# livesense-inc/fanlin-rs

Hardware: AMD Instinct MI355X
Metric: images/sec whole-node (1080p→300×200 resize+encode); p50 per-image ms (higher is better)
Workload: dtype u8 (exact, as f16 subnormals) x the reference's f32 weights as three f16 terms -> f32 sums (vertical, v_mfma_f32_16x16x32_f16); 24-bit fixed-point intermediate (2^-14 steps, three i8 planes) x 24-bit fixed-point weights (2^-24 steps, three i8 digits), eight of the nine digit products -> exact i32 (h

## Files before the change

### fanlin-rs_amd/csrc/fl_jpeg.hip

```cpp
#include <hip/hip_runtime.h>
#include <stdint.h>

#include "fl_jpeg.h"
#include "fl_jpeg_tables.h"
#include "fl_pixel.h"
#include "fl_types.h"

namespace fl {

namespace {


constexpr int32_t F_0_298 = 2446, F_0_390 = 3196, F_0_541 = 4433, F_0_765 = 6270, F_0_899 = 7373, F_1_175 = 9633, F_1_501 = 12299,
                  F_1_847 = 15137, F_1_961 = 16069, F_2_053 = 16819, F_2_562 = 20995, F_3_072 = 25172;

struct Mat8 { int32_t a[8][8]; };

constexpr void fdct_linear(const int32_t in[8], int32_t out[8])
{
    int32_t t0 = in[0] + in[7], t1 = in[1] + in[6], t2 = in[2] + in[5], t3 = in[3] + in[4];
    const int32_t t10 = t0 + t3, t11 = t1 + t2;
    int32_t t12 = t0 - t3, t13 = t1 - t2;
    t0 = in[0] - in[7]; t1 = in[1] - in[6]; t2 = in[2] - in[5]; t3 = in[3] - in[4];
    out[0] = t10 + t11;
    out[4] = t10 - t11;
    int32_t z1 = (t12 + t13) * F_0_541;
    out[2] = z1 + t12 * F_0_765;
    out[6] = z1 - t13 * F_1_847;
    t12 = t0 + t2;
    t13 = t1 + t3;
    z1 = (t12 + t13) * F_1_175;
    t12 = t12 * (-F_0_390) + z1;
    t13 = t13 * (-F_1_961) + z1;
    z1 = (t0 + t3) * (-F_0_899);
    out[1] = t0 * F_1_501 + z1 + t12;
    out[7] = t3 * F_0_298 + z1 + t13;
    z1 = (t1 + t2) * (-F_2_562);
    out[3] = t1 * F_3_072 + z1 + t13;
    out[5] = t2 * F_2_053 + z1 + t12;
}

constexpr Mat8 make_fdct_matrix()
{
    Mat8 m{};
    for (int j = 0; j < 8; ++j) {
        int32_t e[8] = {0, 0, 0, 0, 0, 0, 0, 0}, o[8] = {0, 0, 0, 0, 0, 0, 0, 0};
        e[j] = 1;
        fdct_linear(e, o);
        for (int k = 0; k < 8; ++k) m.a[k][j] = o[k];
    }
    return m;
}

__constant__ Mat8 kFdct = make_fdct_matrix();

constexpr bool fdct_matrix_fits_i16()
{
    const Mat8 m = make_fdct_matrix();
    for (int k = 0; k < 8; ++k)
        for (int j = 0; j < 8; ++j)
            if (m.a[k][j] > 32767 || m.a[k][j] < -32768) return false;
    return true;
}
static_assert(fdct_matrix_fits_i16(), "the passes use v_dot2_i32_i16: matrix entries must be 16-bit");

typedef short i16x2 __attribute__((ext_vector_type(2)));
__device__ __forceinline__ i16x2 as_i16x2(uint32_t v) { return __builtin_bit_cast(i16x2, v); }
__device__ __forceinline__ uint32_t pack_i16(int32_t lo, int32_t hi) { return ((uint32_t)lo & 0xffffu) | ((uint32_t)hi << 16); }
__device__ __forceinline__ int32_t dot8_i16(const uint32_t m[4], const uint4 v)
{
    int32_t p = __builtin_amdgcn_sdot2(as_i16x2(m[0]), as_i16x2(v.x), 0, false);
    p = __builtin_amdgcn_sdot2(as_i16x2(m[1]), as_i16x2(v.y), p, false);
    p = __builtin_amdgcn_sdot2(as_i16x2(m[2]), as_i16x2(v.z), p, false);
    return __builtin_amdgcn_sdot2(as_i16x2(m[3]), as_i16x2(v.w), p, false);
}

struct NaturalOrder { uint8_t n[64]; };
constexpr NaturalOrder make_natural()
{
    NaturalOrder t{};
    for (int k = 0; k < 64; ++k) t.n[k] = kUnzigzag[k];
    return t;
}
__constant__ NaturalOrder kNatural = make_natural();

struct HuffLut { uint32_t e[256]; };

constexpr HuffLut make_lut(const HuffSpec &s)
{
    HuffLut t{};
    uint32_t code = 0;
    int k = 0;
    for (int l = 1; l <= 16; ++l) {
        for (int i = 0; i < s.len[l - 1]; ++i, ++k) t.e[s.val[k]] = ((uint32_t)l << 16) | code++;
        code <<= 1;
    }
    return t;
}

struct HuffAll { HuffLut ac[2], dc[2]; };
constexpr HuffAll make_all() { return HuffAll{{make_lut(kAcLuma), make_lut(kAcChroma)}, {make_lut(kDcLuma), make_lut(kDcChroma)}}; }
__constant__ HuffAll kHuff = make_all();


template <int N>
__device__ __forceinline__ uint32_t dpp_row_shr(uint32_t v)
{
    return (uint32_t)__builtin_amdgcn_update_dpp(0, (int)v, 0x110 + N, 0xf, 0xf, false);
}

__device__ __forceinline__ uint32_t wave_inclusive_scan(uint32_t v, uint32_t lane)
{
    (void)lane;
    v += dpp_row_shr<1>(v);
    v += dpp_row_shr<2>(v);
    v += dpp_row_shr<4>(v);
    v += dpp_row_shr<8>(v);
    v += (uint32_t)__builtin_amdgcn_update_dpp(0, (int)v, 0x142, 0xa, 0xf, false);
    v += (uint32_t)__builtin_amdgcn_update_dpp(0, (int)v, 0x143, 0xc, 0xf, false);
    return v;
}

__device__ __forceinline__ void wave_lds_sync()
{
    __builtin_amdgcn_fence(__ATOMIC_SEQ_CST, "wavefront");
    __builtin_amdgcn_wave_barrier();
}

constexpr uint32_t kPackThreads = 512;
constexpr uint32_t kPackWaves = kPackThreads / 64;

__device__ __forceinline__ uint32_t wg_exclusive_scan(uint32_t v, uint32_t *s_w, uint32_t *total)
{
    const uint32_t lane = threadIdx.x & 63u, wave = threadIdx.x >> 6;
    const uint32_t inc = wave_inclusive_scan(v, lane);
    __syncthreads();
    if (lane == 63u) s_w[wave] = inc;
    __syncthreads();
    uint32_t base = 0, sum = 0;
#pragma unroll
    for (uint32_t i = 0; i < kPackWaves; ++i) { const uint32_t t = s_w[i]; if (i < wave) base += t; sum += t; }
    *total = sum;
    return base + inc - v;
}

__device__ __forceinline__ uint32_t coef_size(int32_t v)
{
    const uint32_t mag = (uint32_t)(v < 0 ? -v : v);
    return mag ? 32u - (uint32_t)__clz(mag) : 0u;
}


#ifndef FL_JPEG_BPW
#define FL_JPEG_BPW 16
#define FL_JPEG_WPG 2
#define FL_JPEG_PREFETCH 3
#endif
constexpr uint32_t kBlocksPerWave = FL_JPEG_BPW;
constexpr uint32_t kWavesPerWg = FL_JPEG_WPG;
constexpr uint32_t kPrefetch = FL_JPEG_PREFETCH;
static_assert(kBlocksPerWave == 32u || kBlocksPerWave == 16u, "the coding phase's lane mapping");
constexpr uint32_t kJpegThreads = 64u * kWavesPerWg;
constexpr uint32_t kBlocksPerWg = kWavesPerWg * kBlocksPerWave;
constexpr uint32_t kUnitsPerWave = 3u * kBlocksPerWave;

static_assert(63u * (16u + 10u) <= kAcWordsPerUnit * 32u, "a unit's AC code must fit its acbits slot");

struct WaveLds {
    int16_t coef[kUnitsPerWave][64];
    uint64_t nz[kUnitsPerWave];
    __attribute__((aligned(16))) int16_t smp[3][64];
    __attribute__((aligned(16))) int16_t p1[3][64];
};

__device__ __forceinline__ void stage_ac_luts(uint32_t *s_ac)
{
    for (uint32_t i = threadIdx.x; i < 512u; i += kJpegThreads) s_ac[i] = kHuff.ac[i >> 8].e[i & 255u];
    __syncthreads();
}

template <bool kRgba>
__device__ __forceinline__ uint32_t block_pixel(const JpegJob &jb, uint32_t brow, uint32_t bcol, uint32_t r, uint32_t c)
{
    uint32_t px = bcol * 8u + c, py = brow * 8u + r;
    px = px < jb.w ? px : jb.w - 1u;
    py = py < jb.h ? py : jb.h - 1u;
    if constexpr (kRgba) return ((const __attribute__((address_space(1))) uint32_t *)jb.src)[(size_t)py * jb.w + px];
    uint32_t pr, pg, pb, pa;
    load_rgba(jb.src + ((size_t)py * jb.w + px) * jb.c, jb.c, pr, pg, pb, pa);
    return pr | (pg << 8) | (pb << 16);
}

__device__ __forceinline__ void dct_quant_block(const uint32_t (&smp)[3], uint32_t nat, uint32_t r, uint32_t c, const uint32_t (&m1)[4],
                                                const uint32_t (&m2)[4], uint4 k1, const uint32_t (&q)[3], const uint32_t (&magic)[3],
                                                WaveLds &w, int32_t (&qv)[3])
{
#pragma unroll
    for (int k = 0; k < 3; ++k) w.smp[k][nat] = (int16_t)smp[k];
    wave_lds_sync();
#pragma unroll
    for (int k = 0; k < 3; ++k) {
        const int32_t p = dot8_i16(m1, *reinterpret_cast<const uint4 *>(w.smp[k] + r * 8));
        const int32_t v1 = ((p << k1.x) + (int32_t)k1.y) >> 11;
        w.p1[k][c * 8 + r] = (int16_t)v1;
    }
    wave_lds_sync();
#pragma unroll
    for (int k = 0; k < 3; ++k) {
        const int32_t p2 = dot8_i16(m2, *reinterpret_cast<const uint4 *>(w.p1[k] + c * 8));
        const int32_t d = (p2 + (int32_t)k1.z) >> k1.w;
        const int32_t sg = d >> 31;
        const uint32_t an = (uint32_t)((d ^ sg) - sg) >> 3;
        const uint32_t rq = __umulhi(2u * an + q[k], magic[k]);
        qv[k] = ((int32_t)rq ^ sg) - sg;
    }
}

typedef __attribute__((address_space(1))) uint32_t global_u32;

struct UnitBits {
    uint64_t acc;
    uint32_t pend, total, wi;
    global_u32 *out;
    __device__ __forceinline__ void put(uint32_t code, uint32_t len)
    {
        acc = (acc << len) | code;
        pend += len;
        total += len;
        if (pend >= 32u) { pend -= 32u; out[wi++] = (uint32_t)(acc >> pend); }
    }
};

template <bool kRgba>
__device__ __forceinline__ void transform_blocks(const JpegJob &jb, const uint32_t *__restrict__ arena, uint32_t first, uint32_t count,
                                                 uint32_t lane, WaveLds &w)
{
    const uint32_t nat = kNatural.n[lane], r = nat >> 3, c = nat & 7u;
    uint32_t m1[4], m2[4];
#pragma unroll
    for (int j = 0; j < 4; ++j) {
        m1[j] = pack_i16(kFdct.a[c][2 * j], kFdct.a[c][2 * j + 1]);
        m2[j] = pack_i16(kFdct.a[r][2 * j], kFdct.a[r][2 * j + 1]);
    }
    const uint8_t *qt = reinterpret_cast<const uint8_t *>(arena + jb.tab_off) + 624;
    const uint32_t *mg = reinterpret_cast<const uint32_t *>(qt + 128);
    const uint32_t q[3] = {qt[nat], qt[64 + nat], qt[64 + nat]};
    const uint32_t magic[3] = {mg[nat], mg[64 + nat], mg[64 + nat]};
    const uint4 k1 = {(c == 0u || c == 4u) ? 13u : 0u, c == 0u ? (uint32_t)(-(8 * 128) * 8192) : (c == 4u ? 0u : 1u << 10),
                      (r == 0u || r == 4u) ? 2u : 1u << 14, (r == 0u || r == 4u) ? 2u : 15u};
    uint32_t brow = first / jb.bx, bcol = first - brow * jb.bx;
    uint32_t ahead[kPrefetch];
#pragma unroll
    for (uint32_t j = 0; j < kPrefetch; ++j) {
        ahead[j] = block_pixel<kRgba>(jb, brow, bcol, r, c);
        if (++bcol == jb.bx) { bcol = 0; ++brow; }
    }
    for (uint32_t i = 0; i < count; ++i) {
        const uint32_t rgb = kRgba ? ahead[0] & 0xffffffu : ahead[0];
#pragma unroll
        for (uint32_t j = 0; j + 1u < kPrefetch; ++j) ahead[j] = ahead[j + 1u];
        ahead[kPrefetch - 1u] = block_pixel<kRgba>(jb, brow, bcol, r, c);
        if (++bcol == jb.bx) { bcol = 0; ++brow; }
        uint32_t smp[3];
        jfif_px(rgb, smp[0], smp[1], smp[2]);
        const bool flat = __ballot(rgb != (uint32_t)__builtin_amdgcn_readfirstlane((int)rgb)) == 0ull;
        if (flat) {
            if (lane == 0u) {
#pragma unroll
                for (int k = 0; k < 3; ++k) {
                    const int32_t d = 64 * ((int32_t)smp[k] - 128);
                    const int32_t sg = d >> 31;
                    const uint32_t an = (uint32_t)((d ^ sg) - sg) >> 3;
                    const uint32_t rq = __umulhi(2u * an + q[k], magic[k]);
                    w.coef[i * 3u + k][0] = (int16_t)(((int32_t)rq ^ sg) - sg);
                    w.nz[i * 3u + k] = 0ull;
                }
            }
            continue;
        }
        int32_t qv[3];
        dct_quant_block(smp, nat, r, c, m1, m2, k1, q, magic, w, qv);
#pragma unroll
        for (int k = 0; k < 3; ++k) {
            w.coef[i * 3u + k][lane] = (int16_t)qv[k];
            const uint64_t nz = __ballot(qv[k] != 0) & ~1ull;
            if (lane == 0u) w.nz[i * 3u + k] = nz;
        }
    }
}

__global__ __launch_bounds__(kJpegThreads) void jpeg_dct_quant_kernel(const JpegJob *__restrict__ jobs, const uint32_t *__restrict__ arena,
                                                                      uint32_t job_base)
{
    __shared__ WaveLds s_w[kWavesPerWg];
    __shared__ uint32_t s_ac[512];
    const JpegJob jb = jobs[job_base + blockIdx.y];
    const uint32_t wave = threadIdx.x >> 6, lane = threadIdx.x & 63u;
    const uint32_t nblocks = jb.bx * jb.by;
    if (blockIdx.x * kBlocksPerWg >= nblocks) return;
    stage_ac_luts(s_ac);
    const uint32_t first = blockIdx.x * kBlocksPerWg + wave * kBlocksPerWave;
    if (first >= nblocks) return;
    const uint32_t count = min(kBlocksPerWave, nblocks - first);
    WaveLds &w = s_w[wave];

    if (jb.c == 4u && (reinterpret_cast<uintptr_t>(jb.src) & 3u) == 0u) transform_blocks<true>(jb, arena, first, count, lane, w);
    else transform_blocks<false>(jb, arena, first, count, lane, w);
    wave_lds_sync();

    uint32_t b, u, u_end;
    bool chroma;
    if constexpr (kBlocksPerWave == 32u) {
        b = lane & 31u;
        chroma = lane >= 32u;
        u = b * 3u + (chroma ? 1u : 0u);
        u_end = b * 3u + (chroma ? 3u : 1u);
    } else {
        b = lane & 15u;
        chroma = lane >= 16u;
        u = b * 3u + (lane >> 4);
        u_end = lane >= 48u ? u : u + 1u;
    }
    if (b >= count) return;
    const uint32_t *tab = s_ac + (chroma ? 256u : 0u);
    const uint32_t eob = tab[0], zrl = tab[0xF0];
    for (; u < u_end; ++u) {
        const uint32_t unit = first * 3u + u;
        const int16_t *cf = w.coef[u];
        uint64_t m = w.nz[u];
        UnitBits ub{0ull, 0u, 0u, unit * kAcWordsPerUnit, (global_u32 *)jb.acbits};
        uint32_t prev = 0;
        uint32_t pos = (uint32_t)__builtin_ctzll(m | (1ull << 63));
        int32_t v = cf[pos];
        while (m) {
            const uint32_t cpos = pos;
            const int32_t cv = v;
            m &= m - 1ull;
            pos = (uint32_t)__builtin_ctzll(m | (1ull << 63));
            v = cf[pos];
            uint32_t run = cpos - prev - 1u;
            prev = cpos;
            while (run > 15u) { ub.put(zrl & 0xffffu, zrl >> 16); run -= 16u; }
            const uint32_t mag = (uint32_t)(cv < 0 ? -cv : cv);
            const uint32_t size = 32u - (uint32_t)__clz(mag);
            const uint32_t value = (uint32_t)(cv + (cv >> 31)) & ((1u << size) - 1u);
            const uint32_t e = tab[(run << 4) | size];
            ub.put(((e & 0xffffu) << size) | value, (e >> 16) + size);
        }
        if (prev != 63u) ub.put(eob & 0xffffu, eob >> 16);
        if (ub.pend) ub.out[ub.wi] = (uint32_t)(ub.acc << (32u - ub.pend));
        jb.meta[unit] = ((uint32_t)(uint16_t)cf[0]) | (ub.total << 16);
    }
}


constexpr uint32_t kWinWords = 8192;

__device__ __forceinline__ void win_or(uint32_t *win, uint32_t wbase, uint64_t g, uint32_t val)
{
    const uint64_t W = g >> 5;
    const uint32_t sh = (uint32_t)g & 31u;
    const uint32_t hi = val >> sh, lo = sh ? val << (32u - sh) : 0u;
    if (hi && W >= wbase && W < (uint64_t)wbase + kWinWords) atomicOr(&win[W - wbase], hi);
    if (lo && W + 1 >= wbase && W + 1 < (uint64_t)wbase + kWinWords) atomicOr(&win[W + 1 - wbase], lo);
}

__device__ __forceinline__ uint32_t dc_code(const JpegJob &jb, uint32_t u, uint32_t meta, uint32_t *len)
{
    const int32_t dc = (int16_t)(meta & 0xffffu), prev = u >= 3u ? (int32_t)(int16_t)(jb.meta[u - 3u] & 0xffffu) : 0;
    const int32_t diff = dc - prev;
    const uint32_t size = coef_size(diff);
    const uint32_t value = (uint32_t)(diff < 0 ? diff - 1 : diff) & ((1u << size) - 1u);
    const uint32_t e = kHuff.dc[(u % 3u) ? 1 : 0].e[size];
    *len = (e >> 16) + size;
    return (((e & 0xffffu) << size) | value) << (32u - *len);
}

__global__ __launch_bounds__(kPackThreads) void jpeg_pack_kernel(const JpegJob *__restrict__ jobs, const uint32_t *__restrict__ arena,
                                                                 uint32_t job_base)
{
    __shared__ uint32_t s_win[kWinWords];
    __shared__ uint32_t s_w[kPackWaves], s_carry, s_lo, s_hi;
    const JpegJob jb = jobs[job_base + blockIdx.x];
    const uint32_t tid = threadIdx.x;
    const uint32_t nunits = jb.bx * jb.by * 3u;
    constexpr uint32_t T = kPackThreads;

    for (uint32_t i = tid; i < kWinWords; i += T) s_win[i] = 0u;
    if (tid == 0u) s_carry = 0u;
    __syncthreads();
    for (uint32_t base = 0; base < nunits; base += T) {
        const uint32_t u = base + tid;
        uint32_t len = 0, dl = 0, dcw = 0, nw = 0, a0 = 0, a1 = 0;
        if (u < nunits) {
            const uint32_t m = jb.meta[u];
            nw = ((m >> 16) + 31u) >> 5;
            if (nw > 0u) a0 = jb.acbits[(size_t)u * kAcWordsPerUnit];
            if (nw > 1u) a1 = jb.acbits[(size_t)u * kAcWordsPerUnit + 1u];
            dcw = dc_code(jb, u, m, &dl);
            len = dl + (m >> 16);
        }
        uint32_t chunk;
        const uint32_t ex = wg_exclusive_scan(len, s_w, &chunk);
        const uint32_t carry = s_carry;
        if (u < nunits) {
            const uint32_t off = carry + ex;
            jb.unit_off[u] = off;
            win_or(s_win, 0u, off, dcw);
            if (nw > 0u) win_or(s_win, 0u, (uint64_t)off + dl, a0);
            if (nw > 1u) win_or(s_win, 0u, (uint64_t)off + dl + 32u, a1);
            for (uint32_t w = 2; w < nw; ++w) win_or(s_win, 0u, (uint64_t)off + dl + 32u * w, jb.acbits[(size_t)u * kAcWordsPerUnit + w]);
        }
        __syncthreads();
        if (tid == 0u) s_carry = carry + chunk;
        __syncthreads();
    }
    const uint32_t total_bits = s_carry;
    if (tid == 0u) jb.unit_off[nunits] = total_bits;
    __threadfence_block();
    __syncthreads();
    const uint32_t nbytes = (total_bits + 7u) >> 3, limit = jb.dst_cap;
    const uint8_t *hdr = reinterpret_cast<const uint8_t *>(arena + jb.tab_off);
    for (uint32_t i = tid; i < kJpegHeaderBytes; i += T) if (i < limit) jb.dst[i] = hdr[i];

    uint32_t ff_before = 0;
    for (uint32_t wbase = 0; wbase * 32ull < total_bits; wbase += kWinWords) {
        const uint64_t wb = (uint64_t)wbase * 32u, we = wb + (uint64_t)kWinWords * 32u;
        if (wbase != 0u) {
            for (uint32_t i = tid; i < kWinWords; i += T) s_win[i] = 0u;
            if (tid == 0u) {
                uint32_t lo = 0, hi = nunits;
                while (lo < hi) { const uint32_t mid = (lo + hi) >> 1; if (jb.unit_off[mid + 1u] > wb) hi = mid; else lo = mid + 1u; }
                s_lo = lo;
                uint32_t lo2 = lo, hi2 = nunits;
                while (lo2 < hi2) { const uint32_t mid = (lo2 + hi2) >> 1; if (jb.unit_off[mid] >= we) hi2 = mid; else lo2 = mid + 1u; }
                s_hi = lo2;
            }
        } else if (tid == 0u) { s_lo = 0u; s_hi = 0u; }
        __syncthreads();
        const uint32_t u_lo = s_lo, u_hi = s_hi;
        for (uint32_t ub = u_lo; ub < u_hi; ub += T / 2u) {
            const uint32_t u = ub + (tid >> 1), j = tid & 1u;
            if (u < u_hi) {
                const uint32_t m = jb.meta[u], off = jb.unit_off[u];
                uint32_t dl;
                const uint32_t dcw = dc_code(jb, u, m, &dl);
                if (j == 0u) win_or(s_win, wbase, off, dcw);
                const uint32_t nw = ((m >> 16) + 31u) >> 5;
                for (uint32_t w = j; w < nw; w += 2u)
                    win_or(s_win, wbase, (uint64_t)off + dl + 32u * w, jb.acbits[(size_t)u * kAcWordsPerUnit + w]);
            }
        }
        __syncthreads();
        if (tid == 0u && (total_bits & 7u) && (total_bits >> 5) >= wbase && (total_bits >> 5) < wbase + kWinWords)
            s_win[(total_bits >> 5) - wbase] |= (0xFFu >> (total_bits & 7u)) << (24u - 8u * ((total_bits >> 3) & 3u));
        __syncthreads();
        const uint32_t win_bytes = (uint32_t)min((uint64_t)kWinWords * 4u, (uint64_t)nbytes - (uint64_t)wbase * 4u);
        if (tid == 0u) s_carry = 0u;
        __syncthreads();
        for (uint32_t base = 0; base < win_bytes; base += 4u * T) {
            const uint32_t i = base + tid * 4u;
            const uint32_t word = i < win_bytes ? s_win[i >> 2] : 0u;
            const uint32_t valid = i < win_bytes ? (win_bytes - i < 4u ? win_bytes - i : 4u) : 0u;
            uint32_t ff = 0;
#pragma unroll
            for (uint32_t k = 0; k < 4; ++k) ff += (k < valid && ((word >> (24u - 8u * k)) & 255u) == 255u) ? 1u : 0u;
            uint32_t chunk;
            const uint32_t ex = wg_exclusive_scan(ff, s_w, &chunk);
            const uint32_t carry = s_carry;
            uint64_t o = (uint64_t)kJpegHeaderBytes + (uint64_t)wbase * 4u + i + ff_before + carry + ex;
#pragma unroll
            for (uint32_t k = 0; k < 4; ++k) {
                if (k < valid) {
                    const uint32_t b = (word >> (24u - 8u * k)) & 255u;
                    if (o < limit) jb.dst[o] = (uint8_t)b;
                    ++o;
                    if (b == 255u) { if (o < limit) jb.dst[o] = 0u; ++o; }
                }
            }
            __syncthreads();
            if (tid == 0u) s_carry = carry + chunk;
            __syncthreads();
        }
        ff_before += s_carry;
        __syncthreads();
    }
    if (tid == 0u) {
        const uint64_t end = (uint64_t)kJpegHeaderBytes + nbytes + ff_before;
        if (end + 2u <= limit) {
            jb.dst[end] = 0xFF; jb.dst[end + 1u] = 0xD9;
            jb.result[1] = (uint32_t)(end + 2u);
        } else {
            jb.result[1] = 0u;
            atomicOr(&jb.result[0], FL_JPEG_RESULT_OVERFLOW);
        }
    }
}

}

hipError_t launch_jpeg_encode(const JpegJob *jobs, const uint32_t *arena, uint32_t job_base, uint32_t njobs, uint32_t max_blocks,
                              hipStream_t st)
{
    if (!njobs || !max_blocks) return hipSuccess;
    hipLaunchKernelGGL(jpeg_dct_quant_kernel, dim3((max_blocks + kBlocksPerWg - 1) / kBlocksPerWg, njobs), dim3(kJpegThreads), 0, st, jobs, arena, job_base);
    FL_LAUNCH_CHECK();
    hipLaunchKernelGGL(jpeg_pack_kernel, dim3(njobs), dim3(kPackThreads), 0, st, jobs, arena, job_base);
    FL_LAUNCH_CHECK();
    return hipSuccess;
}

}
```

Baseline: 555,300.

## Restructure JPEG pack kernel: multi-unit-per-thread scans, fewer barriers, wave-level stuffing

Reworks the pack kernel so each thread handles six units and eight window words per round. Offsets come from wave-level scans, with a single cross-wave LDS exchange per round that uses double-buffered scratch, which removes most workgroup barriers and the tid-0 carry round-trips. It also counts 0xFF bytes with a bit trick, narrows addressing to 32-bit, preloads the DC Huffman tables into LDS, and uses 8-byte AC loads. Units with more than two AC words take a separate slow path. The cost is higher register pressure and more complex lane-to-component mapping logic.

```diff
diff --git a/fanlin-rs_amd/csrc/fl_jpeg.hip b/fanlin-rs_amd/csrc/fl_jpeg.hip
--- a/fanlin-rs_amd/csrc/fl_jpeg.hip
+++ b/fanlin-rs_amd/csrc/fl_jpeg.hip
@@ -130,18 +130,23 @@
 constexpr uint32_t kPackThreads = 512;
 constexpr uint32_t kPackWaves = kPackThreads / 64;
 
-__device__ __forceinline__ uint32_t wg_exclusive_scan(uint32_t v, uint32_t *s_w, uint32_t *total)
+__device__ __forceinline__ void lds_barrier()
+{
+    __builtin_amdgcn_fence(__ATOMIC_RELEASE, "workgroup", "local");
+    __builtin_amdgcn_s_barrier();
+    __builtin_amdgcn_fence(__ATOMIC_ACQUIRE, "workgroup", "local");
+}
+
+__device__ __forceinline__ uint32_t waves_exclusive_scan(uint32_t wave_total, uint32_t *s_w, uint32_t *total)
 {
     const uint32_t lane = threadIdx.x & 63u, wave = threadIdx.x >> 6;
-    const uint32_t inc = wave_inclusive_scan(v, lane);
-    __syncthreads();
-    if (lane == 63u) s_w[wave] = inc;
-    __syncthreads();
+    if (lane == 0u) s_w[wave] = wave_total;
+    lds_barrier();
     uint32_t base = 0, sum = 0;
 #pragma unroll
     for (uint32_t i = 0; i < kPackWaves; ++i) { const uint32_t t = s_w[i]; if (i < wave) base += t; sum += t; }
     *total = sum;
-    return base + inc - v;
+    return base;
 }
 
 __device__ __forceinline__ uint32_t coef_size(int32_t v)
@@ -355,141 +360,232 @@
 
 
 constexpr uint32_t kWinWords = 8192;
-
-__device__ __forceinline__ void win_or(uint32_t *win, uint32_t wbase, uint64_t g, uint32_t val)
-{
-    const uint64_t W = g >> 5;
-    const uint32_t sh = (uint32_t)g & 31u;
+constexpr uint32_t kPackUnitsPerThread = 6;
+constexpr uint32_t kPackWordsPerThread = 8;
+constexpr uint32_t kPackRoundUnits = kPackThreads * kPackUnitsPerThread;
+constexpr uint32_t kPackRoundWords = kPackThreads * kPackWordsPerThread;
+static_assert((64u * kPackUnitsPerThread) % 3u == 0u, "a wave's run of units starts with a Y unit: the component is (step + lane) % 3");
+static_assert(kWinWords % kPackRoundWords == 0u, "the stuffing rounds tile the window");
+static_assert(kAcWordsPerUnit % 2u == 0u, "a unit's first two AC words are one 8-byte load");
+constexpr uint32_t kPackHeaderPerThread = (kJpegHeaderBytes + kPackThreads - 1u) / kPackThreads;
+
+typedef __attribute__((address_space(1))) uint8_t global_u8;
+typedef uint32_t u32x2 __attribute__((ext_vector_type(2)));
+typedef __attribute__((address_space(1))) u32x2 global_u32x2;
+
+__device__ __forceinline__ uint32_t load_u32(const global_u32 *base, uint32_t byte_off)
+{
+    return *(const global_u32 *)((const global_u8 *)base + byte_off);
+}
+__device__ __forceinline__ void store_u32(global_u32 *base, uint32_t byte_off, uint32_t v)
+{
+    *(global_u32 *)((global_u8 *)base + byte_off) = v;
+}
+
+__device__ __forceinline__ void win_or(uint32_t *win, uint32_t wbase, uint32_t g, uint32_t val)
+{
+    const uint32_t W = (g >> 5) - wbase;
+    const uint32_t sh = g & 31u;
     const uint32_t hi = val >> sh, lo = sh ? val << (32u - sh) : 0u;
-    if (hi && W >= wbase && W < (uint64_t)wbase + kWinWords) atomicOr(&win[W - wbase], hi);
-    if (lo && W + 1 >= wbase && W + 1 < (uint64_t)wbase + kWinWords) atomicOr(&win[W + 1 - wbase], lo);
-}
-
-__device__ __forceinline__ uint32_t dc_code(const JpegJob &jb, uint32_t u, uint32_t meta, uint32_t *len)
-{
-    const int32_t dc = (int16_t)(meta & 0xffffu), prev = u >= 3u ? (int32_t)(int16_t)(jb.meta[u - 3u] & 0xffffu) : 0;
+    if (hi && W < kWinWords) atomicOr(&win[W], hi);
+    if (lo && W + 1u < kWinWords) atomicOr(&win[W + 1u], lo);
+}
+
+__device__ __forceinline__ uint32_t dc_code(int32_t dc, int32_t prev, const uint32_t *e, uint32_t *len)
+{
     const int32_t diff = dc - prev;
     const uint32_t size = coef_size(diff);
     const uint32_t value = (uint32_t)(diff < 0 ? diff - 1 : diff) & ((1u << size) - 1u);
-    const uint32_t e = kHuff.dc[(u % 3u) ? 1 : 0].e[size];
-    *len = (e >> 16) + size;
-    return (((e & 0xffffu) << size) | value) << (32u - *len);
-}
-
-__global__ __launch_bounds__(kPackThreads) void jpeg_pack_kernel(const JpegJob *__restrict__ jobs, const uint32_t *__restrict__ arena,
-                                                                 uint32_t job_base)
+    const uint32_t c = e[size];
+    *len = (c >> 16) + size;
+    return (((c & 0xffffu) << size) | value) << (32u - *len);
+}
+
+__device__ __forceinline__ uint32_t count_ff(uint32_t w)
+{
+    const uint32_t x = ~w;
+    return (uint32_t)__popc(~(((x & 0x7f7f7f7fu) + 0x7f7f7f7fu) | x | 0x7f7f7f7fu));
+}
+
+__global__ __launch_bounds__(kPackThreads) __attribute__((amdgpu_waves_per_eu(8, 8)))
+void jpeg_pack_kernel(const JpegJob *__restrict__ jobs, const uint32_t *__restrict__ arena, uint32_t job_base)
 {
     __shared__ uint32_t s_win[kWinWords];
-    __shared__ uint32_t s_w[kPackWaves], s_carry, s_lo, s_hi;
+    __shared__ uint32_t s_scan[2][kPackWaves], s_dc[2][16], s_lo, s_hi;
     const JpegJob jb = jobs[job_base + blockIdx.x];
-    const uint32_t tid = threadIdx.x;
+    const uint32_t tid = threadIdx.x, lane = tid & 63u, wave = tid >> 6;
     const uint32_t nunits = jb.bx * jb.by * 3u;
-    constexpr uint32_t T = kPackThreads;
-
-    for (uint32_t i = tid; i < kWinWords; i += T) s_win[i] = 0u;
-    if (tid == 0u) s_carry = 0u;
-    __syncthreads();
-    for (uint32_t base = 0; base < nunits; base += T) {
-        const uint32_t u = base + tid;
-        uint32_t len = 0, dl = 0, dcw = 0, nw = 0, a0 = 0, a1 = 0;
-        if (u < nunits) {
-            const uint32_t m = jb.meta[u];
-            nw = ((m >> 16) + 31u) >> 5;
-            if (nw > 0u) a0 = jb.acbits[(size_t)u * kAcWordsPerUnit];
-            if (nw > 1u) a1 = jb.acbits[(size_t)u * kAcWordsPerUnit + 1u];
-            dcw = dc_code(jb, u, m, &dl);
-            len = dl + (m >> 16);
+    constexpr uint32_t T = kPackThreads, U = kPackUnitsPerThread, S = kPackWordsPerThread;
+    const global_u32 *meta = (const global_u32 *)jb.meta;
+    const global_u32 *acw = (const global_u32 *)jb.acbits;
+    const global_u32x2 *ac2 = (const global_u32x2 *)jb.acbits;
+    global_u32 *unit_off = (global_u32 *)jb.unit_off;
+    global_u8 *dst = (global_u8 *)jb.dst;
+    const global_u8 *hdr = (const global_u8 *)(arena + jb.tab_off);
+    const uint32_t limit = jb.dst_cap;
+    uint32_t par = 0;
+
+    const uint32_t l3 = lane % 3u;
+    uint32_t carry = 0;
+    for (uint32_t base = 0; base < nunits; base += kPackRoundUnits) {
+        const uint32_t u0 = base + wave * (64u * U) + lane;
+        uint32_t m[U], mp[U];
+        u32x2 a[U];
+#pragma unroll
+        for (uint32_t s = 0; s < U; ++s) {
+            const uint32_t uc = min(u0 + 64u * s, nunits - 1u);
+            m[s] = load_u32(meta, uc * 4u);
+            mp[s] = load_u32(meta, (uc >= 3u ? uc - 3u : 0u) * 4u);
+            a[s] = __builtin_nontemporal_load(&ac2[(size_t)uc * (kAcWordsPerUnit / 2u)]);
+        }
+        if (base == 0u) {
+            for (uint32_t i = tid; i < kWinWords; i += T) s_win[i] = 0u;
+            const uint32_t dc_entry = kHuff.dc[(tid >> 4) & 1u].e[tid & 15u];
+            if (tid < 32u) s_dc[tid >> 4][tid & 15u] = dc_entry;
+            lds_barrier();
+        }
+        uint32_t dcw[U], info[U], ex[U], run = 0;
+        bool longer = false;
+#pragma unroll
+        for (uint32_t s = 0; s < U; ++s) {
+            const uint32_t u = u0 + 64u * s;
+            const bool chroma = l3 != (3u - s % 3u) % 3u;
+            const int32_t prev = u >= 3u ? (int32_t)(int16_t)(mp[s] & 0xffffu) : 0;
+            uint32_t dl;
+            dcw[s] = dc_code((int16_t)(m[s] & 0xffffu), prev, s_dc[chroma ? 1 : 0], &dl);
+            const uint32_t acl = u < nunits ? m[s] >> 16 : 0u;
+            const uint32_t len = u < nunits ? dl + acl : 0u;
+            info[s] = dl | (acl << 8);
+            longer |= acl > 64u;
+            const uint32_t inc = wave_inclusive_scan(len, lane);
+            ex[s] = run + inc - len;
+            run += (uint32_t)__builtin_amdgcn_readlane((int)inc, 63);
+            asm volatile("" : "+v"(dcw[s]), "+v"(info[s]), "+v"(ex[s]));
+            __builtin_amdgcn_sched_barrier(0);
         }
         uint32_t chunk;
-        const uint32_t ex = wg_exclusive_scan(len, s_w, &chunk);
-        const uint32_t carry = s_carry;
-        if (u < nunits) {
-            const uint32_t off = carry + ex;
-            jb.unit_off[u] = off;
-            win_or(s_win, 0u, off, dcw);
-            if (nw > 0u) win_or(s_win, 0u, (uint64_t)off + dl, a0);
-            if (nw > 1u) win_or(s_win, 0u, (uint64_t)off + dl + 32u, a1);
-            for (uint32_t w = 2; w < nw; ++w) win_or(s_win, 0u, (uint64_t)off + dl + 32u * w, jb.acbits[(size_t)u * kAcWordsPerUnit + w]);
-        }
-        __syncthreads();
-        if (tid == 0u) s_carry = carry + chunk;
-        __syncthreads();
-    }
-    const uint32_t total_bits = s_carry;
-    if (tid == 0u) jb.unit_off[nunits] = total_bits;
-    __threadfence_block();
-    __syncthreads();
-    const uint32_t nbytes = (total_bits + 7u) >> 3, limit = jb.dst_cap;
-    const uint8_t *hdr = reinterpret_cast<const uint8_t *>(arena + jb.tab_off);
-    for (uint32_t i = tid; i < kJpegHeaderBytes; i += T) if (i < limit) jb.dst[i] = hdr[i];
+        const uint32_t first = carry + waves_exclusive_scan(run, s_scan[par], &chunk);
+        par ^= 1u;
+#pragma unroll
+        for (uint32_t s = 0; s < U; ++s) {
+            const uint32_t u = u0 + 64u * s;
+            if (u < nunits) {
+                const uint32_t off = first + ex[s], acl = info[s] >> 8, ac_at = off + (info[s] & 255u);
+                store_u32(unit_off, u * 4u, off);
+                win_or(s_win, 0u, off, dcw[s]);
+                if (acl > 0u) win_or(s_win, 0u, ac_at, a[s].x);
+                if (acl > 32u) win_or(s_win, 0u, ac_at + 32u, a[s].y);
+            }
+            __builtin_amdgcn_sched_barrier(0);
+        }
+        if (__any(longer)) {
+            if (longer) {
+#pragma unroll 1
+                for (uint32_t s = 0; s < U; ++s) {
+                    const uint32_t u = u0 + 64u * s;
+                    if (u >= nunits) break;
+                    const uint32_t mu = load_u32(meta, u * 4u), nw = ((mu >> 16) + 31u) >> 5;
+                    if (nw <= 2u) continue;
+                    const int32_t prev = u >= 3u ? (int32_t)(int16_t)(load_u32(meta, (u - 3u) * 4u) & 0xffffu) : 0;
+                    uint32_t dl;
+                    (void)dc_code((int16_t)(mu & 0xffffu), prev, s_dc[(u % 3u) ? 1 : 0], &dl);
+                    const uint32_t ac_at = load_u32(unit_off, u * 4u) + dl;
+                    for (uint32_t w = 2; w < nw; ++w) win_or(s_win, 0u, ac_at + 32u * w, acw[(size_t)u * kAcWordsPerUnit + w]);
+                }
+            }
+        }
+        carry += chunk;
+    }
+    const uint32_t total_bits = carry;
+    if (tid == 0u) store_u32(unit_off, nunits * 4u, total_bits);
+    const uint32_t nbytes = (total_bits + 7u) >> 3, nwords = (nbytes + 3u) >> 2;
+    uint32_t head[kPackHeaderPerThread];
+#pragma unroll
+    for (uint32_t j = 0; j < kPackHeaderPerThread; ++j) head[j] = hdr[min(tid + j * T, kJpegHeaderBytes - 1u)];
 
     uint32_t ff_before = 0;
-    for (uint32_t wbase = 0; wbase * 32ull < total_bits; wbase += kWinWords) {
-        const uint64_t wb = (uint64_t)wbase * 32u, we = wb + (uint64_t)kWinWords * 32u;
+    for (uint32_t wbase = 0; wbase < nwords; wbase += kWinWords) {
         if (wbase != 0u) {
+            __threadfence_block();
+            __syncthreads();
             for (uint32_t i = tid; i < kWinWords; i += T) s_win[i] = 0u;
             if (tid == 0u) {
+                const uint64_t wb = (uint64_t)wbase * 32u, we = wb + (uint64_t)kWinWords * 32u;
                 uint32_t lo = 0, hi = nunits;
-                while (lo < hi) { const uint32_t mid = (lo + hi) >> 1; if (jb.unit_off[mid + 1u] > wb) hi = mid; else lo = mid + 1u; }
+                while (lo < hi) { const uint32_t mid = (lo + hi) >> 1; if (unit_off[mid + 1u] > wb) hi = mid; else lo = mid + 1u; }
                 s_lo = lo;
                 uint32_t lo2 = lo, hi2 = nunits;
-                while (lo2 < hi2) { const uint32_t mid = (lo2 + hi2) >> 1; if (jb.unit_off[mid] >= we) hi2 = mid; else lo2 = mid + 1u; }
+                while (lo2 < hi2) { const uint32_t mid = (lo2 + hi2) >> 1; if (unit_off[mid] >= we) hi2 = mid; else lo2 = mid + 1u; }
                 s_hi = lo2;
             }
-        } else if (tid == 0u) { s_lo = 0u; s_hi = 0u; }
-        __syncthreads();
-        const uint32_t u_lo = s_lo, u_hi = s_hi;
-        for (uint32_t ub = u_lo; ub < u_hi; ub += T / 2u) {
-            const uint32_t u = ub + (tid >> 1), j = tid & 1u;
-            if (u < u_hi) {
-                const uint32_t m = jb.meta[u], off = jb.unit_off[u];
-                uint32_t dl;
-                const uint32_t dcw = dc_code(jb, u, m, &dl);
-                if (j == 0u) win_or(s_win, wbase, off, dcw);
-                const uint32_t nw = ((m >> 16) + 31u) >> 5;
-                for (uint32_t w = j; w < nw; w += 2u)
-                    win_or(s_win, wbase, (uint64_t)off + dl + 32u * w, jb.acbits[(size_t)u * kAcWordsPerUnit + w]);
-            }
-        }
-        __syncthreads();
-        if (tid == 0u && (total_bits & 7u) && (total_bits >> 5) >= wbase && (total_bits >> 5) < wbase + kWinWords)
-            s_win[(total_bits >> 5) - wbase] |= (0xFFu >> (total_bits & 7u)) << (24u - 8u * ((total_bits >> 3) & 3u));
-        __syncthreads();
-        const uint32_t win_bytes = (uint32_t)min((uint64_t)kWinWords * 4u, (uint64_t)nbytes - (uint64_t)wbase * 4u);
-        if (tid == 0u) s_carry = 0u;
-        __syncthreads();
-        for (uint32_t base = 0; base < win_bytes; base += 4u * T) {
-            const uint32_t i = base + tid * 4u;
-            const uint32_t word = i < win_bytes ? s_win[i >> 2] : 0u;
-            const uint32_t valid = i < win_bytes ? (win_bytes - i < 4u ? win_bytes - i : 4u) : 0u;
-            uint32_t ff = 0;
-#pragma unroll
-            for (uint32_t k = 0; k < 4; ++k) ff += (k < valid && ((word >> (24u - 8u * k)) & 255u) == 255u) ? 1u : 0u;
+            lds_barrier();
+            const uint32_t u_lo = s_lo, u_hi = s_hi;
+            for (uint32_t ub = u_lo; ub < u_hi; ub += T / 2u) {
+                const uint32_t u = ub + (tid >> 1), j = tid & 1u;
+                if (u < u_hi) {
+                    const uint32_t mu = meta[u], off = unit_off[u];
+                    const int32_t prev = u >= 3u ? (int32_t)(int16_t)(meta[u - 3u] & 0xffffu) : 0;
+                    uint32_t dlu;
+                    const uint32_t dcu = dc_code((int16_t)(mu & 0xffffu), prev, s_dc[(u % 3u) ? 1 : 0], &dlu);
+                    if (j == 0u) win_or(s_win, wbase, off, dcu);
+                    const uint32_t nw = ((mu >> 16) + 31u) >> 5;
+                    for (uint32_t w = j; w < nw; w += 2u) win_or(s_win, wbase, off + dlu + 32u * w, acw[(size_t)u * kAcWordsPerUnit + w]);
+                }
+            }
+        }
+        if (tid == 0u && (total_bits & 7u) && (total_bits >> 5) - wbase < kWinWords)
+            atomicOr(&s_win[(total_bits >> 5) - wbase], (0xFFu >> (total_bits & 7u)) << (24u - 8u * ((total_bits >> 3) & 3u)));
+        lds_barrier();
+
+        const uint32_t win_bytes = min(kWinWords * 4u, nbytes - wbase * 4u);
+        for (uint32_t rb = 0; rb * 4u < win_bytes; rb += kPackRoundWords) {
+            const uint32_t i0 = rb + wave * (64u * S) + lane;
+            uint32_t mine = 0;
+#pragma unroll
+            for (uint32_t s = 0; s < S; ++s) {
+                const uint32_t i = i0 + 64u * s;
+                mine += i * 4u < win_bytes ? count_ff(s_win[i]) : 0u;
+            }
+            const uint32_t wave_ff = (uint32_t)__builtin_amdgcn_readlane((int)wave_inclusive_scan(mine, lane), 63);
             uint32_t chunk;
-            const uint32_t ex = wg_exclusive_scan(ff, s_w, &chunk);
-            const uint32_t carry = s_carry;
-            uint64_t o = (uint64_t)kJpegHeaderBytes + (uint64_t)wbase * 4u + i + ff_before + carry + ex;
-#pragma unroll
-            for (uint32_t k = 0; k < 4; ++k) {
-                if (k < valid) {
-                    const uint32_t b = (word >> (24u - 8u * k)) & 255u;
-                    if (o < limit) jb.dst[o] = (uint8_t)b;
-                    ++o;
-                    if (b == 255u) { if (o < limit) jb.dst[o] = 0u; ++o; }
+            uint32_t run = ff_before + waves_exclusive_scan(wave_ff, s_scan[par], &chunk);
+            par ^= 1u;
+            if (wbase == 0u && rb == 0u) {
+#pragma unroll
+                for (uint32_t j = 0; j < kPackHeaderPerThread; ++j) {
+                    const uint32_t i = tid + j * T;
+                    if (i < kJpegHeaderBytes && i < limit) dst[i] = (uint8_t)head[j];
                 }
             }
-            __syncthreads();
-            if (tid == 0u) s_carry = carry + chunk;
-            __syncthreads();
-        }
-        ff_before += s_carry;
-        __syncthreads();
+#pragma unroll 1
+            for (uint32_t s = 0; s < S; ++s) {
+                const uint32_t i = (i0 + 64u * s) * 4u;
+                const uint32_t word = i < win_bytes ? s_win[i >> 2] : 0u;
+                const uint32_t ff = count_ff(word);
+                const uint32_t inc = wave_inclusive_scan(ff, lane);
+                if (i < win_bytes) {
+                    const uint32_t valid = min(4u, win_bytes - i);
+                    uint32_t o = kJpegHeaderBytes + wbase * 4u + i + run + inc - ff;
+#pragma unroll
+                    for (uint32_t k = 0; k < 4; ++k) {
+                        if (k < valid) {
+                            const uint32_t b = (word >> (24u - 8u * k)) & 255u;
+                            if (o < limit) dst[o] = (uint8_t)b;
+                            ++o;
+                            if (b == 255u) { if (o < limit) dst[o] = 0u; ++o; }
+                        }
+                    }
+                }
+                run += (uint32_t)__builtin_amdgcn_readlane((int)inc, 63);
+            }
+            ff_before += chunk;
+        }
     }
     if (tid == 0u) {
-        const uint64_t end = (uint64_t)kJpegHeaderBytes + nbytes + ff_before;
+        const uint32_t end = kJpegHeaderBytes + nbytes + ff_before;
         if (end + 2u <= limit) {
-            jb.dst[end] = 0xFF; jb.dst[end + 1u] = 0xD9;
-            jb.result[1] = (uint32_t)(end + 2u);
+            dst[end] = 0xFF; dst[end + 1u] = 0xD9;
+            jb.result[1] = end + 2u;
         } else {
             jb.result[1] = 0u;
             atomicOr(&jb.result[0], FL_JPEG_RESULT_OVERFLOW);
```

New measurement: 544,300. -2.0%, worse.
